# bccp/nbodykit

Measured on AMD Instinct MI355X. Metric: FFTPower_particles_per_s, higher is better.
Workload: dtype f64; 1 GPU; C4; particles=1000020746, nmesh=1024, resampler=cic, interlaced=False, mode=1d, compensated=True, parallelism=slab-dp1

## Files before the change

nbodykit_amd/csrc/nbk_common.h:

```cpp
#pragma once
#include <hip/hip_runtime.h>
#include <cstdint>
#include <cstdio>
#include <cstring>
#include <cmath>

#include "../../include/nbk_hip.h"

extern char nbk_errbuf[1024];

#define NBK_SET_ERR(...) snprintf(nbk_errbuf, sizeof(nbk_errbuf), __VA_ARGS__)

#define NBK_CHECK_HIP(expr)                                               \
    do {                                                                  \
        hipError_t _e = (expr);                                           \
        if (_e != hipSuccess) {                                           \
            NBK_SET_ERR("%s failed: %s (%s:%d)", #expr,                   \
                        hipGetErrorString(_e), __FILE__, __LINE__);       \
            return NBK_ERR_HIP;                                           \
        }                                                                 \
    } while (0)

struct cdouble { double re, im; };

__device__ __forceinline__ cdouble cmul(cdouble a, cdouble b) {
    return {a.re * b.re - a.im * b.im, a.re * b.im + a.im * b.re};
}
__device__ __forceinline__ cdouble cadd(cdouble a, cdouble b) {
    return {a.re + b.re, a.im + b.im};
}
__device__ __forceinline__ cdouble csub(cdouble a, cdouble b) {
    return {a.re - b.re, a.im - b.im};
}
__device__ __forceinline__ cdouble cconj(cdouble a) { return {a.re, -a.im}; }
__device__ __forceinline__ cdouble cscale(cdouble a, double s) {
    return {a.re * s, a.im * s};
}

__device__ __forceinline__ int64_t wrap_generic(int64_t i, int64_t n) {
    i %= n;
    return i < 0 ? i + n : i;
}
__device__ __forceinline__ int64_t wrap_idx(int64_t i, int64_t n) {
    if (__builtin_expect((n & (n - 1)) == 0, 1))
        return i & (n - 1);
    return wrap_generic(i, n);
}

typedef unsigned int nbk_u32x2 __attribute__((ext_vector_type(2)));

__device__ __forceinline__ __amdgpu_buffer_rsrc_t
nbk_buffer_rsrc(const double* base, uint32_t bytes) {
    const uint64_t a = (uint64_t)base;
    const uint64_t lo = (uint32_t)__builtin_amdgcn_readfirstlane((int)a);
    const uint64_t hi =
        (uint32_t)__builtin_amdgcn_readfirstlane((int)(a >> 32));
    return __builtin_amdgcn_make_buffer_rsrc(
        (void*)((hi << 32) | lo), 0,
        __builtin_amdgcn_readfirstlane((int)bytes), 0x00020000);
}

__device__ __forceinline__ double
nbk_buffer_load_f64(__amdgpu_buffer_rsrc_t rsrc, uint32_t off) {
    const nbk_u32x2 v =
        __builtin_amdgcn_raw_buffer_load_b64(rsrc, (int)off, 0, 0);
    return __hiloint2double((int)v.y, (int)v.x);
}

__device__ __forceinline__ double freq_full(int64_t g, int64_t n) {
    const int64_t m = (g < n - n / 2) ? g : g - n;
    return ((double)m * (1.0 / (double)n)) * (double)n;
}
__device__ __forceinline__ double freq_half(int64_t g, int64_t n) {
    return (double)((n % 2 == 0 && g == n / 2) ? -(n / 2) : g);
}

__device__ __forceinline__ void nbk_sync_lds() {
    asm volatile("s_waitcnt lgkmcnt(0)\n\ts_barrier" ::: "memory");
}

__device__ __forceinline__ int nbk_bitrev(int j, int bits) {
    return (int)(__brev((unsigned)j) >> (32 - bits));
}

double* nbk_internal_twiddles(int64_t N);

__device__ __forceinline__ double nbk_comp_factor1(int window,
                                                   int interlaced,
                                                   double wi) {
    if (interlaced) {
        const double s = 0.5 * wi;
        const double sc = (s == 0.0) ? 1.0 : sin(s) / s;
        const double p = (window == NBK_WINDOW_CIC) ? sc * sc
                       : (window == NBK_WINDOW_TSC) ? sc * sc * sc
                                                    : sc * sc * sc * sc;
        return 1.0 / p;
    }
    const double s2 = sin(0.5 * wi) * sin(0.5 * wi);
    double d;
    if (window == NBK_WINDOW_CIC)
        d = 1.0 - 2.0 / 3.0 * s2;
    else if (window == NBK_WINDOW_TSC)
        d = 1.0 - s2 + 2.0 / 15.0 * s2 * s2;
    else
        d = 1.0 - 4.0 / 3.0 * s2 + 2.0 / 5.0 * s2 * s2
            - 4.0 / 315.0 * s2 * s2 * s2;
    return 1.0 / sqrt(d);
}

__device__ __forceinline__ double nbk_comp_factor(int window, int interlaced,
                                                  const double w[3]) {
    double corr = 1.0;
    #pragma unroll
    for (int i = 0; i < 3; i++) {
        if (interlaced) {
            const double s = 0.5 * w[i];
            const double sc = (s == 0.0) ? 1.0 : sin(s) / s;
            const double p = (window == NBK_WINDOW_CIC) ? sc * sc
                           : (window == NBK_WINDOW_TSC) ? sc * sc * sc
                                                        : sc * sc * sc * sc;
            corr /= p;
        } else {
            const double s2 = sin(0.5 * w[i]) * sin(0.5 * w[i]);
            double d;
            if (window == NBK_WINDOW_CIC)
                d = 1.0 - 2.0 / 3.0 * s2;
            else if (window == NBK_WINDOW_TSC)
                d = 1.0 - s2 + 2.0 / 15.0 * s2 * s2;
            else
                d = 1.0 - 4.0 / 3.0 * s2 + 2.0 / 5.0 * s2 * s2
                    - 4.0 / 315.0 * s2 * s2 * s2;
            corr /= sqrt(d);
        }
    }
    return corr;
}
```

nbodykit_amd/csrc/nbk_fft.hip:

```cpp
#include "nbk_common.h"
#include <map>
#include <mutex>

namespace {

std::mutex table_mutex;
std::map<int64_t, double*> twiddle_tables;

bool is_pow2(int64_t n) { return n > 0 && (n & (n - 1)) == 0; }

double* get_twiddles(int64_t N) {
    std::lock_guard<std::mutex> lock(table_mutex);
    auto it = twiddle_tables.find(N);
    if (it != twiddle_tables.end()) return it->second;

    const int64_t m = N / 2 + 1;
    double* host = (double*)malloc(m * 2 * sizeof(double));
    if (!host) return nullptr;
    for (int64_t j = 0; j < m; j++) {
        const double ang = -2.0 * M_PI * (double)j / (double)N;
        host[2 * j] = cos(ang);
        host[2 * j + 1] = sin(ang);
    }
    double* dev = nullptr;
    if (hipMalloc(&dev, m * 2 * sizeof(double)) != hipSuccess) {
        free(host);
        return nullptr;
    }
    if (hipMemcpy(dev, host, m * 2 * sizeof(double),
                  hipMemcpyHostToDevice) != hipSuccess) {
        free(host);
        (void)hipFree(dev);
        return nullptr;
    }
    free(host);
    twiddle_tables[N] = dev;
    return dev;
}

template <bool INV>
__device__ void lds_fft4(cdouble* buf, int m, int TI, int PITCH,
                         const cdouble* __restrict__ table,
                         int mstop) {
    const int T = blockDim.x;
    const int tid = threadIdx.x;
    const int bits = 31 - __clz((unsigned)m);
    int len = 2;
    if (bits & 1) {
        for (int w = tid; w < (m >> 1) * TI; w += T) {
            const int c = w % TI;
            const int j = w / TI;
            const int i0 = (2 * j) * PITCH + c;
            const int i1 = i0 + PITCH;
            const cdouble u = buf[i0];
            const cdouble v = buf[i1];
            buf[i0] = cadd(u, v);
            buf[i1] = csub(u, v);
        }
        nbk_sync_lds();
        len = 4;
    }
    for (; 2 * len <= mstop; len <<= 2) {
        const int h = len >> 1;
        const int tw = m / len;
        for (int w = tid; w < (m >> 2) * TI; w += T) {
            const int c = w % TI;
            const int j = w / TI;
            const int grp = j / h;
            const int pos = j - grp * h;
            const int base = (grp * (len << 1) + pos) * PITCH + c;
            const int s = h * PITCH;
            cdouble w1 = table[pos * tw];
            cdouble w2 = table[2 * pos * tw];
            if (INV) { w1.im = -w1.im; w2.im = -w2.im; }
            const cdouble w3 = cmul(w1, w2);
            const cdouble x0 = buf[base];
            const cdouble x1 = buf[base + s];
            const cdouble x2 = buf[base + 2 * s];
            const cdouble x3 = buf[base + 3 * s];
            const cdouble b1 = cmul(x2, w1);
            const cdouble b2 = cmul(x1, w2);
            const cdouble b3 = cmul(x3, w3);
            const cdouble e0 = cadd(x0, b2);
            const cdouble e1 = csub(x0, b2);
            const cdouble o0 = cadd(b1, b3);
            const cdouble o1 = csub(b1, b3);
            buf[base] = cadd(e0, o0);
            buf[base + 2 * s] = csub(e0, o0);
            const cdouble io1 = INV ? cdouble{-o1.im, o1.re}
                                    : cdouble{o1.im, -o1.re};
            buf[base + s] = cadd(e1, io1);
            buf[base + 3 * s] = csub(e1, io1);
        }
        nbk_sync_lds();
    }
}


__global__ void kfft_r2c_z(const double* __restrict__ real,
                           double* __restrict__ cplx,
                           int64_t nz, double scale,
                           const cdouble* __restrict__ table )
{
    extern __shared__ cdouble buf[];
    const int m = (int)(nz >> 1);
    const int bits = 31 - __clz((unsigned)m);
    const int64_t line = blockIdx.x;

    const cdouble* g = (const cdouble*)(real + line * nz);
    for (int q = threadIdx.x; q < m; q += blockDim.x)
        buf[nbk_bitrev(q, bits)] = g[q];
    __syncthreads();

    lds_fft4<false>(buf, m, 1, 1, table, m);

    cdouble* out = (cdouble*)cplx + line * (m + 1);
    for (int k = threadIdx.x; k <= m; k += blockDim.x) {
        const cdouble Zk = buf[k == m ? 0 : k];
        const cdouble Zm = buf[(m - k) % m];
        const cdouble E = cscale(cadd(Zk, cconj(Zm)), 0.5);
        const cdouble D = csub(Zk, cconj(Zm));
        const cdouble O = {0.5 * D.im, -0.5 * D.re};
        const cdouble X = cadd(E, cmul(table[k], O));
        out[k] = cscale(X, scale);
    }
}

__global__ void kfft_c2r_z(const double* __restrict__ cplx,
                           double* __restrict__ real,
                           int64_t nz,
                           const cdouble* __restrict__ table )
{
    extern __shared__ cdouble smem[];
    const int m = (int)(nz >> 1);
    const int bits = 31 - __clz((unsigned)m);
    cdouble* xin = smem;
    cdouble* buf = smem + (m + 1);
    const int64_t line = blockIdx.x;

    const cdouble* g = (const cdouble*)cplx + line * (m + 1);
    for (int k = threadIdx.x; k <= m; k += blockDim.x) {
        cdouble v = g[k];
        if (k == 0 || k == m) v.im = 0.0;
        xin[k] = v;
    }
    __syncthreads();

    for (int k = threadIdx.x; k < m; k += blockDim.x) {
        const cdouble Xk = xin[k];
        const cdouble Xm = cconj(xin[m - k]);
        const cdouble E = cscale(cadd(Xk, Xm), 0.5);
        const cdouble WO = cscale(csub(Xk, Xm), 0.5);
        const cdouble O = cmul(cconj(table[k]), WO);
        const cdouble Z = {E.re - O.im, E.im + O.re};
        buf[nbk_bitrev(k, bits)] = Z;
    }
    __syncthreads();

    lds_fft4<true>(buf, m, 1, 1, table, m);

    cdouble* out = (cdouble*)(real + line * nz);
    for (int t = threadIdx.x; t < m; t += blockDim.x)
        out[t] = {2.0 * buf[t].re, 2.0 * buf[t].im};
}


template <bool INV>
__global__ void kfft_c_strided(double* __restrict__ data,
                               int nfft, int64_t stride,
                               int64_t ostride, int64_t n_inner,
                               int TI, int tiles,
                               const cdouble* __restrict__ table )
{
    extern __shared__ cdouble buf[];
    const int bits = 31 - __clz((unsigned)nfft);
    const int64_t o = blockIdx.x / tiles;
    const int64_t c0 = (int64_t)(blockIdx.x % tiles) * TI;
    cdouble* g = (cdouble*)data + o * ostride + c0;
    const int ncol = (int)min((int64_t)TI, n_inner - c0);

    const int total = nfft * TI;
    for (int base = 0; base < total; base += (int)blockDim.x * 8) {
        cdouble r[8];
        #pragma unroll
        for (int q = 0; q < 8; q++) {
            const int w = base + q * (int)blockDim.x + (int)threadIdx.x;
            if (w < total) {
                const int c = w % TI;
                r[q] = (c < ncol)
                    ? g[(int64_t)(w / TI) * stride + c]
                    : cdouble{0.0, 0.0};
            }
        }
        #pragma unroll
        for (int q = 0; q < 8; q++) {
            const int w = base + q * (int)blockDim.x + (int)threadIdx.x;
            if (w < total)
                buf[nbk_bitrev(w / TI, bits) * TI + (w % TI)] = r[q];
        }
    }
    __syncthreads();

    lds_fft4<INV>(buf, nfft, TI, TI, table, nfft);

    for (int w = threadIdx.x; w < nfft * TI; w += blockDim.x) {
        const int c = w % TI;
        const int j = w / TI;
        if (c < ncol)
            g[(int64_t)j * stride + c] = buf[j * TI + c];
    }
}

int check_len(int64_t n, const char* who) {
    if (!is_pow2(n) || n < 8 || n > 4096) {
        NBK_SET_ERR("%s: length %lld unsupported (need power of two in "
                    "[8, 4096])", who, (long long)n);
        return NBK_ERR_UNSUPPORTED;
    }
    return NBK_OK;
}

#ifndef NBK_MAX_ELL
#define NBK_MAX_ELL 8
#endif

#define NBK_XBIN_STATIC_LDS 4096

struct XBinArgs {
    int64_t n0, n1, n2;
    int64_t nzh;
    int64_t n_inner;
    int64_t y_off;
    double k0x, k0y, k0z;
    double losx, losy, losz;
    int nx_edges, nmu_edges;
    int nell;
    int ells[NBK_MAX_ELL];
    int win1, interl1;
    int clear_zero;
    double volume;
    double k_lo, k_invd;
    double mu_lo, mu_invd;
    int TI, tiles;
};

__device__ __forceinline__ int digx_guess(const double* __restrict__ e,
                                          int ne, double x, double guess)
{
    int b = (int)guess + 1;
    if (b < 0) b = 0;
    if (b > ne) b = ne;
    while (b > 0 && x < e[b - 1]) b--;
    while (b < ne && e[b] <= x) b++;
    return b;
}

__device__ __forceinline__ int digx(const double* __restrict__ edges,
                                    int nedges, double x) {
    int lo = 0, hi = nedges;
    while (lo < hi) {
        const int mid = (lo + hi) >> 1;
        if (edges[mid] <= x) lo = mid + 1;
        else hi = mid;
    }
    return lo;
}

template <int PHASES, int MAXE, bool IL>
__global__ void kxfft_bin(const double* __restrict__ data,
                          const double* __restrict__ data2, XBinArgs A,
                          const double* __restrict__ k2edges_g,
                          const double* __restrict__ muedges_g,
                          const cdouble* __restrict__ table ,
                          double* __restrict__ gout)
{
    const int NB = (A.nx_edges + 1) * (A.nmu_edges + 1);
    const int nfields = 3 + 2 * A.nell;
    const int n0 = (int)A.n0;
    const int TI = A.TI;
    const int W = TI + 1;
    const int T = blockDim.x;
    const int t = threadIdx.x;
    const int bits = 31 - __clz((unsigned)n0);

    extern __shared__ cdouble smem[];
    cdouble* buf = smem;
    cdouble* buf2 = IL ? smem + (size_t)n0 * W : nullptr;
    cdouble* pxv = IL ? smem + 2 * (size_t)n0 * W : nullptr;
    double* h = (double*)smem
        + 2 * (size_t)n0 * W * (IL ? 2 : 1)
        + (IL ? 2 * (size_t)n0 : 0);
    double* ke = h + (size_t)NB * nfields;
// ... 212 lines not shown

                    atomicAdd(&h[bin], kmag * wgt);
                    atomicAdd(&h[NB + bin], mu * wgt);
                    atomicAdd(&h[2 * NB + bin], wgt);
                    double Pm1 = 0.0, P = 1.0;
                    int e = 0;
                    for (int l = 0; e < A.nell && e < MAXE; l++) {
                        if (l > 0) {
                            const double Pn = ((2 * l - 1) * mu * P
                                               - (l - 1) * Pm1) / l;
                            Pm1 = P;
                            P = Pn;
                        }
                        if (l == A.ells[e]) {
                            double wr = vre * P;
                            if (nonsingular)
                                wr = (l % 2) ? 0.0 : 2.0 * wr;
                            atomicAdd(&h[(3 + 2 * e) * NB + bin],
                                      wr * (2.0 * l + 1.0));
                            e++;
                        }
                    }
                }
            }
        }
        nbk_sync_lds();
    }
#undef XBIN_SETUP
#undef XBIN_LOAD
#undef XBIN_STORE
    nbk_sync_lds();
    for (int i = t; i < NB * nfields; i += T)
        if (h[i] != 0.0) atomicAdd(&gout[i], h[i]);
}

}

extern "C" int nbk_fft_r2c_z(const double* real, double* cplx,
                             int64_t nlines, int64_t nz, double scale,
                             void* stream)
{
    int rc = check_len(nz, "nbk_fft_r2c_z");
    if (rc) return rc;
    if (nlines == 0) return NBK_OK;
    double* table = get_twiddles(nz);
    if (!table) { NBK_SET_ERR("twiddle alloc failed"); return NBK_ERR_HIP; }
    const int block = (int)std::min<int64_t>(512, nz / 4);
    const size_t shmem = (size_t)(nz / 2) * sizeof(cdouble);
    hipLaunchKernelGGL(kfft_r2c_z, dim3((uint32_t)nlines), dim3(block), shmem,
                       (hipStream_t)stream, real, cplx, nz, scale,
                       (const cdouble*)table);
    NBK_CHECK_HIP(hipGetLastError());
    return NBK_OK;
}

extern "C" int nbk_fft_c2r_z(const double* cplx, double* real,
                             int64_t nlines, int64_t nz, void* stream)
{
    int rc = check_len(nz, "nbk_fft_c2r_z");
    if (rc) return rc;
    if (nlines == 0) return NBK_OK;
    double* table = get_twiddles(nz);
    if (!table) { NBK_SET_ERR("twiddle alloc failed"); return NBK_ERR_HIP; }
    const int block = (int)std::min<int64_t>(512, nz / 4);
    const size_t shmem = (size_t)(nz + 1) * sizeof(cdouble);
    hipLaunchKernelGGL(kfft_c2r_z, dim3((uint32_t)nlines), dim3(block), shmem,
                       (hipStream_t)stream, cplx, real, nz,
                       (const cdouble*)table);
    NBK_CHECK_HIP(hipGetLastError());
    return NBK_OK;
}

extern "C" int nbk_fft_c_strided(double* cplx, int64_t nfft, int64_t stride,
                                 int64_t n_outer, int64_t outer_stride,
                                 int64_t n_inner, int sign, void* stream)
{
    int rc = check_len(nfft, "nbk_fft_c_strided");
    if (rc) return rc;
    if (n_outer == 0 || n_inner == 0) return NBK_OK;
    double* table = get_twiddles(2 * nfft);
    if (!table) { NBK_SET_ERR("twiddle alloc failed"); return NBK_ERR_HIP; }

    static int TI0 = 0;
    if (!TI0) {
        const char* e = getenv("NBK_FFT_TI");
        TI0 = e ? atoi(e) : 4;
        if (TI0 < 1 || TI0 > 16) TI0 = 4;
    }
    int TI = TI0;
    const int64_t lds_cap = (TI0 != 4) ? 160 * 1024 : 65536;
    while ((int64_t)nfft * TI * (int64_t)sizeof(cdouble) > lds_cap && TI > 1)
        TI >>= 1;
    if (TI > n_inner) TI = (int)n_inner;
    const int tiles = (int)((n_inner + TI - 1) / TI);
    const int64_t grid = n_outer * tiles;
    if (grid > 0x7fffffff) {
        NBK_SET_ERR("nbk_fft_c_strided: grid too large");
        return NBK_ERR_ARG;
    }
    static int block = 0;
    if (!block) {
        const char* e = getenv("NBK_FFT_BLOCK");
        block = e ? atoi(e) : 1024;
        if (block < 64 || block > 1024) block = 1024;
    }
    const size_t shmem = (size_t)nfft * TI * sizeof(cdouble);
    if (shmem > 65536) {
        static size_t raised_fwd = 0, raised_inv = 0;
        size_t& raised = (sign < 0) ? raised_fwd : raised_inv;
        if (shmem > raised) {
            (void)hipFuncSetAttribute(
                sign < 0
                    ? reinterpret_cast<const void*>(&kfft_c_strided<false>)
                    : reinterpret_cast<const void*>(&kfft_c_strided<true>),
                hipFuncAttributeMaxDynamicSharedMemorySize, (int)shmem);
            raised = shmem;
        }
    }

    if (sign < 0)
        hipLaunchKernelGGL(kfft_c_strided<false>, dim3((uint32_t)grid),
                           dim3(block), shmem, (hipStream_t)stream,
                           cplx, (int)nfft, stride, outer_stride, n_inner,
                           TI, tiles, (const cdouble*)table);
    else
        hipLaunchKernelGGL(kfft_c_strided<true>, dim3((uint32_t)grid),
                           dim3(block), shmem, (hipStream_t)stream,
                           cplx, (int)nfft, stride, outer_stride, n_inner,
                           TI, tiles, (const cdouble*)table);
    NBK_CHECK_HIP(hipGetLastError());
    return NBK_OK;
}

extern "C" int nbk_fft_x_bin_f64(const double* data, const double* data2,
                                 const int64_t nmesh[3],
                                 int64_t n_inner, int64_t y_off,
                                 const double box[3],
                                 int window1, int interlaced1,
                                 int clear_zero, double volume,
                                 const double* k2edges, int64_t nx_edges,
                                 const double* muedges, int64_t nmu_edges,
                                 const double dig_hints[4],
                                 const double los[3],
                                 const int* ells, int nell,
                                 double* out_sums, void* stream)
{
    const bool il = data2 != nullptr;
    int rc = check_len(nmesh[0], "nbk_fft_x_bin_f64");
    if (rc) return rc;
    if (n_inner == 0) return NBK_OK;
    if (nell > NBK_MAX_ELL) {
        NBK_SET_ERR("nbk_fft_x_bin_f64: at most %d multipoles",
                    NBK_MAX_ELL);
        return NBK_ERR_ARG;
    }
    if (window1 > 2) {
        NBK_SET_ERR("nbk_fft_x_bin_f64: bad window %d", window1);
        return NBK_ERR_ARG;
    }
    double* table = get_twiddles(2 * nmesh[0]);
    if (!table) { NBK_SET_ERR("twiddle alloc failed"); return NBK_ERR_HIP; }

    XBinArgs A;
    A.n0 = nmesh[0]; A.n1 = nmesh[1]; A.n2 = nmesh[2];
    A.nzh = nmesh[2] / 2 + 1;
    A.n_inner = n_inner;
    A.y_off = y_off;
    A.k0x = 2.0 * M_PI / box[0];
    A.k0y = 2.0 * M_PI / box[1];
    A.k0z = 2.0 * M_PI / box[2];
    A.losx = los[0]; A.losy = los[1]; A.losz = los[2];
    A.nx_edges = (int)nx_edges;
    A.nmu_edges = (int)nmu_edges;
    A.nell = nell;
    for (int e = 0; e < NBK_MAX_ELL; e++)
        A.ells[e] = e < nell ? ells[e] : -1;
    A.win1 = window1;
    A.interl1 = interlaced1;
    A.clear_zero = clear_zero;
    A.volume = volume;
    A.k_lo = dig_hints[0];
    A.k_invd = dig_hints[1];
    A.mu_lo = dig_hints[2];
    A.mu_invd = dig_hints[3];

    const int64_t NB = (nx_edges + 1) * (nmu_edges + 1);
    const int nfields = 3 + 2 * nell;
    const size_t fixed = ((size_t)NB * nfields + nx_edges + nmu_edges
                          + nmesh[0]) * sizeof(double);
    static int TI0 = 0;
    if (!TI0) {
        const char* e = getenv("NBK_XBIN_TI");
        TI0 = e ? atoi(e) : 4;
        if (TI0 < 1 || TI0 > 16) TI0 = 4;
    }
    int TI = TI0;
    const int64_t regcap = il ? 2 * 1024 : 4 * 1024;
    while (TI > 1 && (int64_t)nmesh[0] * TI > regcap)
        TI >>= 1;
    const size_t fixed_il = fixed
        + (il ? (size_t)nmesh[0] * sizeof(cdouble) : 0);
    const int nbufs = il ? 2 : 1;
    const size_t lds_budget = 160 * 1024 - NBK_XBIN_STATIC_LDS;
// ... 106 lines not shown
```

nbodykit_amd/csrc/nbk_paint.hip:

```cpp
#include "nbk_common.h"
#include <type_traits>

namespace {

__device__ __forceinline__ void merged_deposit(double* __restrict__ mesh,
                                               long long addr, double val,
                                               int lane) {
    const long long a_up1 = __shfl_up(addr, 1, 64);
    const bool head = (lane == 0) || (a_up1 != addr);
    const unsigned long long heads = __ballot(head);
    const unsigned long long below = heads
        & (~0ULL >> (63 - lane));
    const int myhead = 63 - __clzll(below);
    #pragma unroll
    for (int d = 1; d < 64; d <<= 1) {
        const double v_up = __shfl_up(val, d, 64);
        if (lane - d >= myhead) val += v_up;
    }
    const bool next_head = ((lane < 63)
                            && ((heads >> (lane + 1)) & 1ULL));
    if (addr >= 0 && (lane == 63 || next_head))
        atomicAdd(&mesh[addr], val);
}

constexpr int WINDOW_NNB = 3;

template <int WINDOW>
constexpr int window_support() {
    return (WINDOW == NBK_WINDOW_CIC) ? 2
         : (WINDOW == NBK_WINDOW_TSC) ? 3 : 4;
}

template <int WINDOW>
__device__ __forceinline__ int64_t base_cell(double u) {
    const double f = floor(WINDOW == NBK_WINDOW_TSC ? u + 0.5 : u);
    return (int64_t)f - (WINDOW == NBK_WINDOW_CIC ? 0 : 1);
}

template <int WINDOW, int SUP>
__device__ __forceinline__ void paint_weights(double u0, double u1,
                                              double u2,
                                              double (&w0)[SUP],
                                              double (&w1)[SUP],
                                              double (&w2)[SUP],
                                              int64_t& b0, int64_t& b1,
                                              int64_t& b2) {
    if (WINDOW == NBK_WINDOW_CIC) {
        const double f0 = floor(u0), f1 = floor(u1), f2 = floor(u2);
        b0 = base_cell<WINDOW>(u0); b1 = base_cell<WINDOW>(u1);
        b2 = base_cell<WINDOW>(u2);
        w0[SUP - 1] = u0 - f0; w0[0] = 1.0 - (u0 - f0);
        w1[SUP - 1] = u1 - f1; w1[0] = 1.0 - (u1 - f1);
        w2[SUP - 1] = u2 - f2; w2[0] = 1.0 - (u2 - f2);
    } else if (WINDOW == NBK_WINDOW_TSC) {
        const double f0 = floor(u0 + 0.5), f1 = floor(u1 + 0.5),
                     f2 = floor(u2 + 0.5);
        b0 = base_cell<WINDOW>(u0); b1 = base_cell<WINDOW>(u1);
        b2 = base_cell<WINDOW>(u2);
        #pragma unroll
        for (int d = 0; d < 3; d++) {
            const double s0 = u0 - (f0 + d - 1);
            const double s1 = u1 - (f1 + d - 1);
            const double s2 = u2 - (f2 + d - 1);
            const double a0 = fabs(s0), a1 = fabs(s1), a2 = fabs(s2);
            w0[d] = a0 < 0.5 ? 0.75 - s0 * s0
                             : 0.5 * (1.5 - a0) * (1.5 - a0);
            w1[d] = a1 < 0.5 ? 0.75 - s1 * s1
                             : 0.5 * (1.5 - a1) * (1.5 - a1);
            w2[d] = a2 < 0.5 ? 0.75 - s2 * s2
                             : 0.5 * (1.5 - a2) * (1.5 - a2);
        }
    } else {
        const double f0 = floor(u0), f1 = floor(u1), f2 = floor(u2);
        b0 = base_cell<WINDOW>(u0); b1 = base_cell<WINDOW>(u1);
        b2 = base_cell<WINDOW>(u2);
        #pragma unroll
        for (int d = 0; d < 4; d++) {
            const double s0 = fabs(u0 - (f0 + d - 1));
            const double s1 = fabs(u1 - (f1 + d - 1));
            const double s2 = fabs(u2 - (f2 + d - 1));
            w0[d] = s0 < 1.0
                ? (4.0 - 6.0 * s0 * s0 + 3.0 * s0 * s0 * s0) / 6.0
                : (2.0 - s0) * (2.0 - s0) * (2.0 - s0) / 6.0;
// ... 91 lines not shown
        const double u1 = py[i] * invH1 + shift;
        const int b0 = (int)base_cell<WINDOW>(u0);
        const int b1 = (int)base_cell<WINDOW>(u1);
        mn0 = min(mn0, b0); mx0 = max(mx0, b0);
        mn1 = min(mn1, b1); mx1 = max(mx1, b1);
    }
    atomicMin(&s_min0, mn0); atomicMax(&s_max0, mx0);
    atomicMin(&s_min1, mn1); atomicMax(&s_max1, mx1);
    __syncthreads();

    const int wx = s_max0 - s_min0 + SUP;
    const int wy = s_max1 - s_min1 + SUP;
    const int64_t cells = (int64_t)wx * wy * n2;
    const bool use_lds = (ibeg < iend) && cells > 0
        && cells <= NBK_TILE_MAX_CELLS;

    if (!use_lds) {
        for (int64_t i = ibeg + threadIdx.x; i < iend; i += blockDim.x) {
            const double u0 = px[i] * invH0 + shift;
            const double u1 = py[i] * invH1 + shift;
            const double u2 = pz[i] * invH2 + shift;
            const double m = mass ? mass[i] : 1.0;
            double w0[SUP], w1[SUP], w2[SUP];
            int64_t b0, b1, b2;
            paint_weights<WINDOW, SUP>(u0, u1, u2, w0, w1, w2, b0, b1, b2);
            for (int dx = 0; dx < SUP; dx++) {
                const int64_t gx = wrap_idx(b0 + dx, n0);
                if (gx < x0 || gx >= x0 + nx_local) continue;
                for (int dy = 0; dy < SUP; dy++) {
                    const int64_t gy = wrap_idx(b1 + dy, n1);
                    const double wxy = w0[dx] * w1[dy] * m;
                    for (int dz = 0; dz < SUP; dz++) {
                        const int64_t gz = wrap_idx(b2 + dz, n2);
                        atomicAdd(&mesh[((gx - x0) * n1 + gy) * n2 + gz],
                                  wxy * w2[dz]);
                    }
                }
            }
        }
        return;
    }

    for (int64_t w = threadIdx.x; w < cells; w += blockDim.x)
        buf[w] = 0.0;
    __syncthreads();

    for (int64_t i = ibeg + threadIdx.x; i < iend; i += blockDim.x) {
        const double u0 = px[i] * invH0 + shift;
        const double u1 = py[i] * invH1 + shift;
        const double u2 = pz[i] * invH2 + shift;
        const double m = mass ? mass[i] : 1.0;
        double w0[SUP], w1[SUP], w2[SUP];
        int64_t b0, b1, b2;
        paint_weights<WINDOW, SUP>(u0, u1, u2, w0, w1, w2, b0, b1, b2);
        const int lx = (int)(b0 - s_min0);
        const int ly = (int)(b1 - s_min1);
        for (int dx = 0; dx < SUP; dx++) {
            for (int dy = 0; dy < SUP; dy++) {
                const double wxy = w0[dx] * w1[dy] * m;
                const int64_t base =
                    ((int64_t)(lx + dx) * wy + (ly + dy)) * n2;
                for (int dz = 0; dz < SUP; dz++) {
                    const int64_t gz = wrap_idx(b2 + dz, n2);
                    unsafeAtomicAdd(&buf[base + gz], wxy * w2[dz]);
                }
            }
        }
    }
    __syncthreads();

    for (int64_t w = threadIdx.x; w < cells; w += blockDim.x) {
        const double v = buf[w];
        if (v == 0.0) continue;
        const int64_t gz = w % n2;
        const int64_t wyidx = (w / n2) % wy;
        const int64_t wxidx = w / ((int64_t)n2 * wy);
        const int64_t gx = wrap_idx(s_min0 + wxidx, n0);
        if (gx < x0 || gx >= x0 + nx_local) continue;
        const int64_t gy = wrap_idx(s_min1 + wyidx, n1);
        atomicAdd(&mesh[((gx - x0) * n1 + gy) * n2 + gz], v);
    }
}

typedef double nbk_f64x2 __attribute__((ext_vector_type(2)));

__device__ __forceinline__ cdouble zfft_ld(const cdouble* z, int i) {
    const nbk_f64x2 v = *reinterpret_cast<const nbk_f64x2*>(z + i);
    return {v.x, v.y};
}
__device__ __forceinline__ void zfft_st(cdouble* z, int i, cdouble a) {
    const nbk_f64x2 v = {a.re, a.im};
    *reinterpret_cast<nbk_f64x2*>(z + i) = v;
}

template <int R>
__device__ __forceinline__ void zfft_butterfly(cdouble (&v)[R]) {
    static_assert(R == 1 || R == 2 || R == 4 || R == 8, "radix");
    if constexpr (R == 2) {
        const cdouble a = v[0], b = v[1];
        v[0] = cadd(a, b);
        v[1] = csub(a, b);
    } else if constexpr (R == 4) {
        const cdouble s0 = cadd(v[0], v[2]), s1 = csub(v[0], v[2]);
        const cdouble s2 = cadd(v[1], v[3]), s3 = csub(v[1], v[3]);
        const cdouble is3 = {s3.im, -s3.re};
        v[0] = cadd(s0, s2);
        v[1] = cadd(s1, is3);
        v[2] = csub(s0, s2);
        v[3] = csub(s1, is3);
    } else if constexpr (R == 8) {
        cdouble e[4] = {v[0], v[2], v[4], v[6]};
        cdouble o[4] = {v[1], v[3], v[5], v[7]};
        zfft_butterfly<4>(e);
        zfft_butterfly<4>(o);
        constexpr double h = 0.70710678118654752440;
        o[1] = {(o[1].re + o[1].im) * h, (o[1].im - o[1].re) * h};
        o[2] = {o[2].im, -o[2].re};
        o[3] = {(o[3].im - o[3].re) * h, -(o[3].re + o[3].im) * h};
        #pragma unroll
        for (int k = 0; k < 4; k++) {
            v[k] = cadd(e[k], o[k]);
            v[k + 4] = csub(e[k], o[k]);
        }
    }
}

struct zfft_twiddles {
    cdouble w1[3];
    cdouble w2[3];
};

template <int N>
__device__ __forceinline__ void zfft_twiddle(cdouble (&v)[N],
                                             const cdouble (&p)[3]) {
    v[1] = cmul(v[1], p[0]);
    if constexpr (N > 2) {
        const cdouble p3 = cmul(p[0], p[1]);
        v[2] = cmul(v[2], p[1]);
        v[3] = cmul(v[3], p3);
        if constexpr (N > 4) {
            v[4] = cmul(v[4], p[2]);
            v[5] = cmul(v[5], cmul(p[0], p[2]));
            v[6] = cmul(v[6], cmul(p[1], p[2]));
            v[7] = cmul(v[7], cmul(p3, p[2]));
        }
    }
}

template <int LOGM>
__device__ __forceinline__ void zfft_load_twiddles(
    zfft_twiddles& tw, const cdouble* __restrict__ table , int lane)
{
    constexpr int R = 1 << (LOGM - 6), m = 64 * R;
    auto W = [&](int e) -> cdouble {
        const cdouble w = table[e > m ? e - m : e];
        return e > m ? cdouble{-w.re, -w.im} : w;
    };
    #pragma unroll
    for (int i = 0; i < 3; i++) {
        if ((1 << i) < R) tw.w1[i] = W(2 * lane << i);
        tw.w2[i] = W(2 * R * (lane & 7) << i);
    }
}

template <int LOGM>
__device__ __forceinline__ void zfft_row(cdouble* z, int lane,
                                         zfft_twiddles tw)
{
    constexpr int R = 1 << (LOGM - 6), L2 = 8 * R;
    asm volatile("" : "+v"(lane));
    #pragma unroll
    for (int i = 0; i < 3; i++) {
        if ((1 << i) < R)
            asm volatile("" : "+v"(tw.w1[i].re), "+v"(tw.w1[i].im));
        asm volatile("" : "+v"(tw.w2[i].re), "+v"(tw.w2[i].im));
    }
    if constexpr (R > 1) {
        cdouble v[R];
        #pragma unroll
        for (int j = 0; j < R; j++) v[j] = zfft_ld(z, lane + 64 * j);
        zfft_butterfly<R>(v);
        zfft_twiddle<R>(v, tw.w1);
        __builtin_amdgcn_wave_barrier();
        #pragma unroll
        for (int k1 = 0; k1 < R; k1++)
            zfft_st(z, 64 * k1 + (lane ^ (8 * ((k1 >> 1) & 1))), v[k1]);
        __builtin_amdgcn_wave_barrier();
    }
    const bool active = (L2 == 64) || lane < L2;
    if (active) {
        const int k1 = lane >> 3, b = lane & 7;
        const int base = 64 * k1 + (b ^ (8 * ((k1 >> 1) & 1)));
        cdouble u[8];
        #pragma unroll
        for (int a = 0; a < 8; a++) u[a] = zfft_ld(z, base ^ (8 * a));
        zfft_butterfly<8>(u);
        zfft_twiddle<8>(u, tw.w2);
        #pragma unroll
        for (int d = 0; d < 8; d++)
            zfft_st(z, L2 * b + ((R * d + k1) ^ b), u[d]);
    }
    __builtin_amdgcn_wave_barrier();
    if (active) {
        cdouble s[8];
        #pragma unroll
        for (int b = 0; b < 8; b++) s[b] = zfft_ld(z, L2 * b + (lane ^ b));
        zfft_butterfly<8>(s);
        #pragma unroll
        for (int c = 0; c < 8; c++) zfft_st(z, lane + L2 * c, s[c]);
    }
    __builtin_amdgcn_wave_barrier();
}

template <int WINDOW, bool DOFFT, int PT, int ZF>
__global__ void kpaint_gather(const double* __restrict__ px,
                              const double* __restrict__ py,
                              const double* __restrict__ pz,
                              const double* __restrict__ mass, int64_t n,
                              int64_t n0, int64_t n1, int64_t n2,
                              double invH0, double invH1, double invH2,
                              double shift,
                              const int* __restrict__ rowtab,
                              double* __restrict__ mesh,
                              int64_t x0, int64_t nx_local,
                              int RG, int P, int xlo, int xhi,
                              int accumulate,
                              const cdouble* __restrict__ table ,
                              double scale,
                              int gs,
                              int phases )
// ... 641 lines not shown
```

Before: 22.89 billion particles/s.

## Add register/LDS column FFT kernel with persistent grid and prefetched loads

Adds a new strided column FFT kernel (kfft_col) for power-of-two sizes 64 to 1024. It runs a persistent grid where each block handles a contiguous range of 4-column tiles. The FFT is split into a register radix-R stage and two LDS radix-8 stages with swizzled slots, and the next tile's global load is issued with 128-bit buffer loads before the current tile is finished. The aim is to cut LDS round-trips and latency compared with the generic lds_fft4 path, which reloads every column through LDS. In exchange it adds complexity, a fixed grid size, env switches including a debug no-FFT mode, and the FFT helpers move into a shared header.

```diff
diff --git a/nbodykit_amd/csrc/nbk_common.h b/nbodykit_amd/csrc/nbk_common.h
--- a/nbodykit_amd/csrc/nbk_common.h
+++ b/nbodykit_amd/csrc/nbk_common.h
@@ -65,6 +65,24 @@
     const nbk_u32x2 v =
         __builtin_amdgcn_raw_buffer_load_b64(rsrc, (int)off, 0, 0);
     return __hiloint2double((int)v.y, (int)v.x);
+}
+
+typedef unsigned int nbk_u32x4 __attribute__((ext_vector_type(4)));
+typedef double nbk_f64x2_bits __attribute__((ext_vector_type(2)));
+
+__device__ __forceinline__ cdouble
+nbk_buffer_load_c128(__amdgpu_buffer_rsrc_t rsrc, uint32_t off) {
+    const nbk_u32x4 v =
+        __builtin_amdgcn_raw_buffer_load_b128(rsrc, (int)off, 0, 0);
+    const nbk_f64x2_bits d = __builtin_bit_cast(nbk_f64x2_bits, v);
+    return {d.x, d.y};
+}
+__device__ __forceinline__ void
+nbk_buffer_store_c128(__amdgpu_buffer_rsrc_t rsrc, uint32_t off,
+                      double re, double im) {
+    const nbk_f64x2_bits d = {re, im};
+    __builtin_amdgcn_raw_buffer_store_b128(
+        __builtin_bit_cast(nbk_u32x4, d), rsrc, (int)off, 0, 0);
 }
 
 __device__ __forceinline__ double freq_full(int64_t g, int64_t n) {
diff --git a/nbodykit_amd/csrc/nbk_fft.hip b/nbodykit_amd/csrc/nbk_fft.hip
--- a/nbodykit_amd/csrc/nbk_fft.hip
+++ b/nbodykit_amd/csrc/nbk_fft.hip
@@ -1,4 +1,5 @@
 #include "nbk_common.h"
+#include "nbk_zfft.h"
 #include <map>
 #include <mutex>
 
@@ -165,7 +166,7 @@
 }
 
 
-template <bool INV>
+template <bool INV, bool NET = true>
 __global__ void kfft_c_strided(double* __restrict__ data,
                                int nfft, int64_t stride,
                                int64_t ostride, int64_t n_inner,
@@ -201,13 +202,153 @@
     }
     __syncthreads();
 
-    lds_fft4<INV>(buf, nfft, TI, TI, table, nfft);
+    if (NET)
+        lds_fft4<INV>(buf, nfft, TI, TI, table, nfft);
 
     for (int w = threadIdx.x; w < nfft * TI; w += blockDim.x) {
         const int c = w % TI;
         const int j = w / TI;
         if (c < ncol)
             g[(int64_t)j * stride + c] = buf[j * TI + c];
+    }
+}
+
+#define NBK_FFTCOL_THREADS 256
+#define NBK_FFTCOL_GRID 2048
+
+template <int LOGN, bool NET>
+__global__ void __launch_bounds__(NBK_FFTCOL_THREADS, 2)
+kfft_col(double* __restrict__ data, int64_t stride, int64_t ostride,
+         int64_t n_inner, int tiles ,
+         int64_t ntiles , double sgn,
+         const cdouble* __restrict__ table )
+{
+    constexpr int R = 1 << (LOGN - 6);
+    constexpr int P = R > 8 ? R / 8 : 1;
+    constexpr int ACT = 8 * R;
+    extern __shared__ cdouble smem[];
+    cdouble* z = smem;
+    const int tid = threadIdx.x, c = tid & 3, l = tid >> 2;
+    const int a = l >> 3, b = l & 7;
+    const bool act = ACT >= 64 || l < ACT;
+
+    cdouble w1[4], w2[3];
+    #pragma unroll
+    for (int i = 0; i < 4; i++)
+        if ((1 << i) < R) w1[i] = table[(2 * l) << i];
+    #pragma unroll
+    for (int i = 0; i < 3; i++) w2[i] = table[(2 * R * b) << i];
+
+    const int64_t chunk = (ntiles + gridDim.x - 1) / gridDim.x;
+    int64_t t = (int64_t)blockIdx.x * chunk;
+    const int64_t tend = t + chunk < ntiles ? t + chunk : ntiles;
+    if (t >= tend) return;
+    int64_t o = t / tiles;
+    int ti = (int)(t - o * tiles);
+
+    auto slot = [&](int q, int x) { return 4 * (8 * q + (x ^ (q & 7))) + c; };
+
+    constexpr uint32_t RANGE = 0x80000000u;
+    const uint32_t off = 16u * ((uint32_t)l * (uint32_t)stride
+                                + (uint32_t)c);
+    auto rowrsrc = [&](int64_t o_, int ti_, int row) {
+        return nbk_buffer_rsrc(
+            data + 2 * (o_ * ostride + 4 * (int64_t)ti_ + row * stride),
+            RANGE);
+    };
+
+    auto maskoff = [&](int ti_, bool on) {
+        return (on & (c < n_inner - 4 * (int64_t)ti_)) ? off : RANGE;
+    };
+    auto load = [&](cdouble (&x)[R], int64_t o_, int ti_, uint32_t loff) {
+        #pragma unroll
+        for (int j = 0; j < R; j++)
+            x[j] = nbk_buffer_load_c128(rowrsrc(o_, ti_, 64 * j), loff);
+    };
+
+    auto run = [&](cdouble (&x)[R], cdouble (&nx)[R]) -> bool {
+        int64_t o2 = o;
+        int ti2 = ti + 1;
+        if (ti2 == tiles) { ti2 = 0; o2++; }
+        const bool more = t + 1 < tend;
+        if (!more) { o2 = o; ti2 = ti; }
+        const uint32_t loff = maskoff(ti2, more);
+        const uint32_t soff = maskoff(ti, true);
+        if constexpr (!NET) {
+            load(nx, o2, ti2, loff);
+            #pragma unroll
+            for (int j = 0; j < R; j++)
+                nbk_buffer_store_c128(rowrsrc(o, ti, 64 * j), soff,
+                                      x[j].re, x[j].im);
+        } else {
+            #pragma unroll
+            for (int i = 0; i < 4; i++)
+                if ((1 << i) < R)
+                    asm volatile("" : "+v"(w1[i].re), "+v"(w1[i].im));
+            #pragma unroll
+            for (int i = 0; i < 3; i++)
+                asm volatile("" : "+v"(w2[i].re), "+v"(w2[i].im));
+            #pragma unroll
+            for (int j = 0; j < R; j++) x[j].im *= sgn;
+            if constexpr (R > 1) {
+                zfft_butterfly<R>(x);
+                zfft_twiddle<R>(x, w1);
+            }
+            __builtin_amdgcn_sched_barrier(0);
+            load(nx, o2, ti2, loff);
+            #pragma unroll
+            for (int k1 = 0; k1 < R; k1++)
+                zfft_st(z, slot(R * a + k1, b), x[k1]);
+            nbk_sync_lds();
+            if (act) {
+                #pragma unroll
+                for (int p = 0; p < P; p++) {
+                    const int k1 = (l >> 3) + 8 * p;
+                    cdouble u[8];
+                    #pragma unroll
+                    for (int a2 = 0; a2 < 8; a2++)
+                        u[a2] = zfft_ld(z, slot(R * a2 + k1, b));
+                    zfft_butterfly<8>(u);
+                    zfft_twiddle<8>(u, w2);
+                    #pragma unroll
+                    for (int d = 0; d < 8; d++)
+                        zfft_st(z, slot(R * d + k1, b), u[d]);
+                    __builtin_amdgcn_sched_barrier(0);
+                }
+            }
+            nbk_sync_lds();
+            if (act) {
+                #pragma unroll
+                for (int p = 0; p < P; p++) {
+                    cdouble s[8];
+                    #pragma unroll
+                    for (int b2 = 0; b2 < 8; b2++)
+                        s[b2] = zfft_ld(z, slot(l + 64 * p, b2));
+                    zfft_butterfly<8>(s);
+                    #pragma unroll
+                    for (int e = 0; e < 8; e++)
+                        nbk_buffer_store_c128(
+                            rowrsrc(o, ti, 64 * p + ACT * e), soff,
+                            s[e].re, s[e].im * sgn);
+                    __builtin_amdgcn_sched_barrier(0);
+                }
+            }
+            nbk_sync_lds();
+        }
+        t++;
+        o = o2;
+        ti = ti2;
+        return more;
+    };
+
+    cdouble A[R], B[R];
+    load(A, o, ti, maskoff(ti, true));
+    #pragma unroll
+    for (int j = 0; j < (NET ? 8 * P : R); j++)
+        nbk_buffer_store_c128(rowrsrc(o, ti, j), RANGE, 0.0, 0.0);
+    for (;;) {
+        if (!run(A, B)) break;
+        if (!run(B, A)) break;
     }
 }
 
@@ -586,11 +727,58 @@
     if (!table) { NBK_SET_ERR("twiddle alloc failed"); return NBK_ERR_HIP; }
 
     static int TI0 = 0;
+    static bool tuned = false;
     if (!TI0) {
         const char* e = getenv("NBK_FFT_TI");
         TI0 = e ? atoi(e) : 4;
         if (TI0 < 1 || TI0 > 16) TI0 = 4;
-    }
+        tuned = e || getenv("NBK_FFT_BLOCK");
+    }
+    static int phases = 0, use_col = 0;
+    if (!phases) {
+        const char* e = getenv("NBK_FFT_PHASES");
+        phases = (e && atoi(e) == 0) ? 2 : 3;
+        e = getenv("NBK_FFT_COL");
+        use_col = !(e && atoi(e) == 0);
+    }
+    const bool net = phases & 1;
+
+    if (use_col && !tuned && nfft >= 64 && nfft <= 1024
+        && stride > 0 && stride <= (1 << 21)) {
+        const int64_t tiles = (n_inner + 3) / 4;
+        if (tiles > 0x7fffffff || n_outer > INT64_MAX / tiles) {
+            NBK_SET_ERR("nbk_fft_c_strided: grid too large");
+            return NBK_ERR_ARG;
+        }
+        const int64_t ntiles = n_outer * tiles;
+        const uint32_t g = (uint32_t)std::min<int64_t>(ntiles,
+                                                       NBK_FFTCOL_GRID);
+        const size_t lds = (size_t)nfft * 4 * sizeof(cdouble);
+        const double sgn = sign < 0 ? 1.0 : -1.0;
+#define NBK_FFTCOL_LAUNCH(LOGN_, NET_)                                     \
+        hipLaunchKernelGGL((kfft_col<LOGN_, NET_>), dim3(g),               \
+                           dim3(NBK_FFTCOL_THREADS), lds,                  \
+                           (hipStream_t)stream, cplx, stride,              \
+                           outer_stride, n_inner, (int)tiles, ntiles,      \
+                           sgn, (const cdouble*)table)
+#define NBK_FFTCOL_CASE(LOGN_)                                             \
+        case 1 << LOGN_:                                                   \
+            if (net) { NBK_FFTCOL_LAUNCH(LOGN_, true); }                   \
+            else { NBK_FFTCOL_LAUNCH(LOGN_, false); }                      \
+            break;
+        switch ((int)nfft) {
+        NBK_FFTCOL_CASE(6)
+        NBK_FFTCOL_CASE(7)
+        NBK_FFTCOL_CASE(8)
+        NBK_FFTCOL_CASE(9)
+        NBK_FFTCOL_CASE(10)
+        }
+#undef NBK_FFTCOL_CASE
+#undef NBK_FFTCOL_LAUNCH
+        NBK_CHECK_HIP(hipGetLastError());
+        return NBK_OK;
+    }
+
     int TI = TI0;
     const int64_t lds_cap = (TI0 != 4) ? 160 * 1024 : 65536;
     while ((int64_t)nfft * TI * (int64_t)sizeof(cdouble) > lds_cap && TI > 1)
@@ -622,7 +810,18 @@
         }
     }
 
-    if (sign < 0)
+    if (!net) {
+        if (shmem > 65536) {
+            NBK_SET_ERR("nbk_fft_c_strided: NBK_FFT_PHASES=0 needs a tile "
+                        "within 64 KiB of LDS");
+            return NBK_ERR_UNSUPPORTED;
+        }
+        hipLaunchKernelGGL((kfft_c_strided<false, false>),
+                           dim3((uint32_t)grid), dim3(block), shmem,
+                           (hipStream_t)stream, cplx, (int)nfft, stride,
+                           outer_stride, n_inner, TI, tiles,
+                           (const cdouble*)table);
+    } else if (sign < 0)
         hipLaunchKernelGGL(kfft_c_strided<false>, dim3((uint32_t)grid),
                            dim3(block), shmem, (hipStream_t)stream,
                            cplx, (int)nfft, stride, outer_stride, n_inner,
diff --git a/nbodykit_amd/csrc/nbk_paint.hip b/nbodykit_amd/csrc/nbk_paint.hip
--- a/nbodykit_amd/csrc/nbk_paint.hip
+++ b/nbodykit_amd/csrc/nbk_paint.hip
@@ -1,4 +1,5 @@
 #include "nbk_common.h"
+#include "nbk_zfft.h"
 #include <type_traits>
 
 namespace {
@@ -256,70 +257,11 @@
     }
 }
 
-typedef double nbk_f64x2 __attribute__((ext_vector_type(2)));
-
-__device__ __forceinline__ cdouble zfft_ld(const cdouble* z, int i) {
-    const nbk_f64x2 v = *reinterpret_cast<const nbk_f64x2*>(z + i);
-    return {v.x, v.y};
-}
-__device__ __forceinline__ void zfft_st(cdouble* z, int i, cdouble a) {
-    const nbk_f64x2 v = {a.re, a.im};
-    *reinterpret_cast<nbk_f64x2*>(z + i) = v;
-}
-
-template <int R>
-__device__ __forceinline__ void zfft_butterfly(cdouble (&v)[R]) {
-    static_assert(R == 1 || R == 2 || R == 4 || R == 8, "radix");
-    if constexpr (R == 2) {
-        const cdouble a = v[0], b = v[1];
-        v[0] = cadd(a, b);
-        v[1] = csub(a, b);
-    } else if constexpr (R == 4) {
-        const cdouble s0 = cadd(v[0], v[2]), s1 = csub(v[0], v[2]);
-        const cdouble s2 = cadd(v[1], v[3]), s3 = csub(v[1], v[3]);
-        const cdouble is3 = {s3.im, -s3.re};
-        v[0] = cadd(s0, s2);
-        v[1] = cadd(s1, is3);
-        v[2] = csub(s0, s2);
-        v[3] = csub(s1, is3);
-    } else if constexpr (R == 8) {
-        cdouble e[4] = {v[0], v[2], v[4], v[6]};
-        cdouble o[4] = {v[1], v[3], v[5], v[7]};
-        zfft_butterfly<4>(e);
-        zfft_butterfly<4>(o);
-        constexpr double h = 0.70710678118654752440;
-        o[1] = {(o[1].re + o[1].im) * h, (o[1].im - o[1].re) * h};
-        o[2] = {o[2].im, -o[2].re};
-        o[3] = {(o[3].im - o[3].re) * h, -(o[3].re + o[3].im) * h};
-        #pragma unroll
-        for (int k = 0; k < 4; k++) {
-            v[k] = cadd(e[k], o[k]);
-            v[k + 4] = csub(e[k], o[k]);
-        }
-    }
-}
 
 struct zfft_twiddles {
     cdouble w1[3];
     cdouble w2[3];
 };
-
-template <int N>
-__device__ __forceinline__ void zfft_twiddle(cdouble (&v)[N],
-                                             const cdouble (&p)[3]) {
-    v[1] = cmul(v[1], p[0]);
-    if constexpr (N > 2) {
-        const cdouble p3 = cmul(p[0], p[1]);
-        v[2] = cmul(v[2], p[1]);
-        v[3] = cmul(v[3], p3);
-        if constexpr (N > 4) {
-            v[4] = cmul(v[4], p[2]);
-            v[5] = cmul(v[5], cmul(p[0], p[2]));
-            v[6] = cmul(v[6], cmul(p[1], p[2]));
-            v[7] = cmul(v[7], cmul(p3, p[2]));
-        }
-    }
-}
 
 template <int LOGM>
 __device__ __forceinline__ void zfft_load_twiddles(
diff --git a/nbodykit_amd/csrc/nbk_zfft.h b/nbodykit_amd/csrc/nbk_zfft.h
--- /dev/null
+++ b/nbodykit_amd/csrc/nbk_zfft.h
@@ -0,0 +1,99 @@
+#pragma once
+#include "nbk_common.h"
+
+typedef double nbk_f64x2 __attribute__((ext_vector_type(2)));
+
+__device__ __forceinline__ cdouble zfft_ld(const cdouble* z, int i) {
+    const nbk_f64x2 v = *reinterpret_cast<const nbk_f64x2*>(z + i);
+    return {v.x, v.y};
+}
+__device__ __forceinline__ void zfft_st(cdouble* z, int i, cdouble a) {
+    const nbk_f64x2 v = {a.re, a.im};
+    *reinterpret_cast<nbk_f64x2*>(z + i) = v;
+}
+
+template <int R>
+__device__ __forceinline__ void zfft_butterfly(cdouble (&v)[R]) {
+    static_assert(R == 1 || R == 2 || R == 4 || R == 8 || R == 16,
+                  "radix");
+    if constexpr (R == 2) {
+        const cdouble a = v[0], b = v[1];
+        v[0] = cadd(a, b);
+        v[1] = csub(a, b);
+    } else if constexpr (R == 4) {
+        const cdouble s0 = cadd(v[0], v[2]), s1 = csub(v[0], v[2]);
+        const cdouble s2 = cadd(v[1], v[3]), s3 = csub(v[1], v[3]);
+        const cdouble is3 = {s3.im, -s3.re};
+        v[0] = cadd(s0, s2);
+        v[1] = cadd(s1, is3);
+        v[2] = csub(s0, s2);
+        v[3] = csub(s1, is3);
+    } else if constexpr (R == 8) {
+        cdouble e[4] = {v[0], v[2], v[4], v[6]};
+        cdouble o[4] = {v[1], v[3], v[5], v[7]};
+        zfft_butterfly<4>(e);
+        zfft_butterfly<4>(o);
+        constexpr double h = 0.70710678118654752440;
+        o[1] = {(o[1].re + o[1].im) * h, (o[1].im - o[1].re) * h};
+        o[2] = {o[2].im, -o[2].re};
+        o[3] = {(o[3].im - o[3].re) * h, -(o[3].re + o[3].im) * h};
+        #pragma unroll
+        for (int k = 0; k < 4; k++) {
+            v[k] = cadd(e[k], o[k]);
+            v[k + 4] = csub(e[k], o[k]);
+        }
+    } else if constexpr (R == 16) {
+        cdouble e[8], o[8];
+        #pragma unroll
+        for (int k = 0; k < 8; k++) {
+            e[k] = v[2 * k];
+            o[k] = v[2 * k + 1];
+        }
+        zfft_butterfly<8>(e);
+        zfft_butterfly<8>(o);
+        constexpr double h = 0.70710678118654752440;
+        constexpr double C = 0.92387953251128675613;
+        constexpr double S = 0.38268343236508977173;
+        o[1] = cmul(o[1], cdouble{C, -S});
+        o[2] = {(o[2].re + o[2].im) * h, (o[2].im - o[2].re) * h};
+        o[3] = cmul(o[3], cdouble{S, -C});
+        o[4] = {o[4].im, -o[4].re};
+        o[5] = cmul(o[5], cdouble{-S, -C});
+        o[6] = {(o[6].im - o[6].re) * h, -(o[6].re + o[6].im) * h};
+        o[7] = cmul(o[7], cdouble{-C, -S});
+        #pragma unroll
+        for (int k = 0; k < 8; k++) {
+            v[k] = cadd(e[k], o[k]);
+            v[k + 8] = csub(e[k], o[k]);
+        }
+    }
+}
+
+template <int N, int NP>
+__device__ __forceinline__ void zfft_twiddle(cdouble (&v)[N],
+                                             const cdouble (&p)[NP]) {
+    static_assert(N <= 8 || NP >= 4, "w^8 needed beyond 8 points");
+    v[1] = cmul(v[1], p[0]);
+    if constexpr (N > 2) {
+        const cdouble p3 = cmul(p[0], p[1]);
+        v[2] = cmul(v[2], p[1]);
+        v[3] = cmul(v[3], p3);
+        if constexpr (N > 4) {
+            v[4] = cmul(v[4], p[2]);
+            v[5] = cmul(v[5], cmul(p[0], p[2]));
+            v[6] = cmul(v[6], cmul(p[1], p[2]));
+            v[7] = cmul(v[7], cmul(p3, p[2]));
+            if constexpr (N > 8) {
+                const cdouble p12 = cmul(p[2], p[3]);
+                v[8] = cmul(v[8], p[3]);
+                v[9] = cmul(v[9], cmul(p[0], p[3]));
+                v[10] = cmul(v[10], cmul(p[1], p[3]));
+                v[11] = cmul(v[11], cmul(p3, p[3]));
+                v[12] = cmul(v[12], p12);
+                v[13] = cmul(v[13], cmul(p[0], p12));
+                v[14] = cmul(v[14], cmul(p[1], p12));
+                v[15] = cmul(v[15], cmul(p3, p12));
+            }
+        }
+    }
+}
```

After: 22.97 billion particles/s, median of 6. No clear change (+0.3%).
